# matteofox/MC-ALF

Hardware: AMD Instinct MI355X
Metric: component-pixel Voigt evals/s (sum_s ncomp_s * npix / t), logL batch on MI355X: `value` with the inputs resident in HBM when the timed region starts, `value_host_api` through the host-pointer entry with P in and logL out inside every step (higher is better)
Workload: dtype f64

## Files before the change

mc-alf_amd/csrc/kernels.hip:

```cpp
#include <hip/hip_runtime.h>

#include <cmath>

#include "kernel_args.h"
#include "voigt_device.h"

namespace mcalf {

__device__ __forceinline__ int xcd_raw() { return (int)(__builtin_amdgcn_s_getreg((3 << 11) | 20) & 15); }
__device__ __forceinline__ int xcd_id() { return (int)(__builtin_amdgcn_s_getreg((3 << 11) | 20) & (kXcds - 1)); }

__device__ __forceinline__ int tile_pos(int i) { return (i & 7) * kPlaneStride + (i >> 3); }

template <int kCtrl, int kRowMask = 0xF>
__device__ __forceinline__ double dpp_move(double v) {
    const unsigned long long u = __builtin_bit_cast(unsigned long long, v);
    const int lo = __builtin_amdgcn_update_dpp(0, (int)(unsigned)u, kCtrl, kRowMask, 0xF, false);
    const int hi = __builtin_amdgcn_update_dpp(0, (int)(unsigned)(u >> 32), kCtrl, kRowMask, 0xF, false);
    return __builtin_bit_cast(double, ((unsigned long long)(unsigned)hi << 32) | (unsigned)lo);
}

__device__ __forceinline__ double wave_sum_to_last(double v) {
    v += dpp_move<0x111>(v);
    v += dpp_move<0x112>(v);
// ... 507 lines not shown
        }
        __syncthreads();
        const int c = sClaim[0], cnt = sClaim[1];
        const bool ok = sClaim[2] != 0;
        __syncthreads();
        if (cnt == 0) {
            if (!rest && dedicated) { rest = true; continue; }
            break;
        }
        if (a.Pdev && ok) {
            const int perBlock = 8 * a.ndim, n = cnt * perBlock;
            for (int i0 = tid; i0 < n; i0 += 4 * kBlock) {
                double v[4];
                size_t at[4];
#pragma unroll
                for (int k = 0; k < 4; ++k) {
                    const int i = i0 + k * kBlock, blk = i / perBlock;
                    at[k] = (size_t)stream_row(x, 8 * (c + blk), nx) * a.ndim + (size_t)(i - blk * perBlock);
                    v[k] = (i < n && at[k] < (size_t)a.nrows * a.ndim) ? a.P[at[k]] : 0.0;
                }
#pragma unroll
                for (int k = 0; k < 4; ++k)
                    if (i0 + k * kBlock < n && at[k] < (size_t)a.nrows * a.ndim) a.Pdev[at[k]] = v[k];
            }
            stream_stores_done();
            __syncthreads();
        }
        for (int k = 0; k < cnt; ++k) {
            const int r = stream_row(x, 8 * (c + k) + wave, nx);
            if (r >= a.nrows) continue;
            SampleHdr* hdrp = reinterpret_cast<SampleHdr*>(reinterpret_cast<double*>(a.hdr) + (size_t)r * a.hdr_stride);
            if (ok) {
                setup_sample<kZeroPad>(as, (long)r, lane, a.recs + (size_t)r * a.rec_stride, a.taps + (size_t)r * a.tap_stride, true, hdrp, true,
                                       kSelfHalo, ends);
            } else if (lane == 0) {
                SampleHdr h;
                h.cont = 0.0; h.bot = 1.0; h.ncl = 0; h.n = 0; h.bad = 1; h.ngeneral = 0;
                *hdrp = h;
            }
        }
        stream_stores_done();
        if (lane < cnt) {
            const int r = stream_row(x, 8 * (c + lane) + wave, nx);
            if (r < a.nrows) __hip_atomic_store(a.ready + r, a.gen, __ATOMIC_RELAXED, __HIP_MEMORY_SCOPE_AGENT);
        }
    }
    __builtin_amdgcn_s_setprio(0);
    __syncthreads();
}

__device__ __forceinline__ void stream_exit(const KArgs& a, int tid) {
    if (tid != 0) return;
    stream_stores_done();
    if (atomicAdd(&a.sctl->exited, 1u) == gridDim.x - 1) {
        unsigned lo = ~0u, hi = 0u;
        for (int k = 0; k < kXcds; ++k) {
            const unsigned n = __hip_atomic_load(&a.sctl->arrive[k], __ATOMIC_RELAXED, __HIP_MEMORY_SCOPE_AGENT);
            lo = min(lo, n); hi = max(hi, n);
        }
        __hip_atomic_store(a.status + 2, lo, __ATOMIC_RELAXED, __HIP_MEMORY_SCOPE_SYSTEM);
        __hip_atomic_store(a.status + 3, hi, __ATOMIC_RELAXED, __HIP_MEMORY_SCOPE_SYSTEM);
        for (int k = 0; k < kXcds; ++k) {
            __hip_atomic_store(&a.sctl->arrive[k], 0u, __ATOMIC_RELAXED, __HIP_MEMORY_SCOPE_AGENT);
            __hip_atomic_store(&a.sctl->sq_eager[k], 0u, __ATOMIC_RELAXED, __HIP_MEMORY_SCOPE_AGENT);
            __hip_atomic_store(&a.sctl->sq_rest[k], 0u, __ATOMIC_RELAXED, __HIP_MEMORY_SCOPE_AGENT);
            __hip_atomic_store(&a.sctl->queue[k], 0u, __ATOMIC_RELAXED, __HIP_MEMORY_SCOPE_AGENT);
        }
        __hip_atomic_store(&a.sctl->exited, 0u, __ATOMIC_RELAXED, __HIP_MEMORY_SCOPE_AGENT);
        stream_stores_done();
        __hip_atomic_store(a.status + 1, a.gen, __ATOMIC_RELAXED, __HIP_MEMORY_SCOPE_SYSTEM);
    }
}

struct ItemLoads {
    double treg[(VT_NY * VT_NTOT + kBlock - 1) / kBlock];
    double rreg[2];
    double tapreg;
    double nu[kPpt];
    double nuNode;
    unsigned long long tileMask;
    SampleHdr hd;
};

template <bool kZeroPad, bool selfHalo, bool kInline, bool kCoh = false>
__device__ __forceinline__ void request_item(const KArgs& a, int w, int tid, ItemLoads& L) {
    asm volatile("" : "+v"(tid));
    constexpr int kTRegs = (VT_NY * VT_NTOT + kBlock - 1) / kBlock;
    constexpr int kRecRegs = 2;
    const int recTotal = a.ncl_cap * kRecStride, tapTotal = 2 * a.n_cap + 8;
    const int s = w / a.ntiles;
    const int tileIdx = w - s * a.ntiles;
#pragma unroll
    for (int i = 0; i < kTRegs; ++i) {
        const int idx = tid + i * kBlock;
        L.treg[i] = (idx < VT_NY * VT_NTOT) ? a.tabs[idx] : 0.0;
    }
    if (!kInline) {
        const double* gr = a.recs + (size_t)s * (kCoh ? a.rec_stride : recTotal);
        const double* gt = a.taps + (kCoh ? (size_t)s * a.tap_stride : (a.taps_shared ? 0 : (size_t)s * tapTotal));
        L.hd = kCoh ? *reinterpret_cast<const SampleHdr*>(reinterpret_cast<const double*>(a.hdr) + (size_t)s * a.hdr_stride) : a.hdr[s];
#pragma unroll
        for (int i = 0; i < kRecRegs; ++i) L.rreg[i] = (tid + i * kBlock < recTotal) ? gr[tid + i * kBlock] : 0.0;
        L.tapreg = (tid < tapTotal) ? gt[tid] : 0.0;
    }
    const int t0 = tileIdx * a.tile;
    const int ext0 = selfHalo ? 0 : t0 - a.n_cap;
    int npixW = a.npix;
    asm volatile("" : "+s"(npixW));
#pragma unroll
    for (int j = 0; j < kPpt; ++j) {
        int e = ext0 + tid + j * kBlock;
        if (!selfHalo && (e < 0 || e >= a.npix)) {
            if (kZeroPad) e = 0;
            else { e %= npixW; if (e < 0) e += npixW; }
        }
        L.nu[j] = a.nu[e];
    }
    L.nuNode = 0.0;
    L.tileMask = 0;
    if (kFarInterp && selfHalo && !kInline) {
        const int wv = tid >> 6, ln = tid & 63;
        L.nuNode = a.nu[kBlock * wv + 64 * (ln >> 3) + VT_INTERP_NODES[ln & 7]];
    } else if (kFarInterp) {
        const int wv = tid >> 6, ln = tid & 63;
        int e = ext0 + 64 * wv + kBlock * (ln >> 3) + VT_INTERP_NODES[ln & 7];
        if (!selfHalo && (e < 0 || e >= a.npix)) { e %= npixW; if (e < 0) e += npixW; }
        L.nuNode = a.nu[e];
        L.tileMask = a.segok[tileIdx];
    }
}

template <bool kZeroPad, bool kSelfHalo, int kLinesPerSync, bool kInline, bool kStream>
__device__ __forceinline__ void fused_items(const KArgs& a, double* smem) {
    double* sTab = smem;
    double* sRec = sTab + 2 * kLinesPerSync * kTabPad;
    double* sW = sRec + a.ncl_cap * kRecStride;
    double* sRed = sW + (2 * a.n_cap + 8);
    double* sWt = sRed + kRedDoubles;
    double* sF = sWt + 64 * VT_INODES;
    int* sNext = reinterpret_cast<int*>(sRed + 3 * kWaves);

    const int tid0 = threadIdx.x;
    double* sT = sF;
    constexpr int kTRegs = (VT_NY * VT_NTOT + kBlock - 1) / kBlock;
    constexpr int kRecRegs = 2;
    constexpr bool selfHalo = kSelfHalo;
    constexpr bool kPreMask = kSelfHalo && !kInline;
    static_assert(kLinesPerSync * kTabPad >= kBlock, "the node sums fit the idle half of the folded tables");
    if (kFarInterp) sWt[(tid0 & 7) * 64 + (tid0 >> 3)] = a.wtab[tid0];
    const int recTotal = a.ncl_cap * kRecStride, tapTotal = 2 * a.n_cap + 8;
    const int xcd = kStream ? xcd_id() : 0;
    const int nItems = kStream ? stream_rows_of(a.nrows, xcd, kXcds) * a.ntiles : a.nitems;

    constexpr bool kOrdered = kSelfHalo && !kInline && !kStream;
    auto item_of = [&](int t) -> int {
        if (kStream) { const int j = t / a.ntiles; return stream_row(xcd, j, kXcds) * a.ntiles + (t - j * a.ntiles); }
        return (kOrdered && a.order) ? a.order[t] : t;
    };
    constexpr bool kDeferTicket = kOrdered || kStream;
    int w;
    unsigned int* const queue = kStream ? &a.sctl->queue[xcd] : a.queue;
    const int firstTickets = kStream ? 0 : (int)gridDim.x;
    if (kStream) {
        if (tid0 == 0) sNext[0] = (int)atomicAdd(queue, 1u);
        __syncthreads();
        const int t = sNext[0];
        __syncthreads();
        if (t >= nItems) {
            stream_exit(a, tid0);
            return;
        }
        w = item_of(t);
        stream_wait_ready(a, w / a.ntiles, 0u);
    } else {
        w = item_of(blockIdx.x);
    }
    ItemLoads L;
    request_item<kZeroPad, kSelfHalo, kInline, kStream>(a, w, tid0, L);

    while (true) {
        int tid = tid0;
        asm volatile("" : "+v"(tid));
        const bool hasCoef = tid < VT_NTOT;
        const int coefPos = tid + (tid >= VT_Z0_OFF ? 1 : 0) + (tid >= VT_ZF_OFF ? 1 : 0);
        const bool coreCoef = tid < VT_NCORE;
        const int s = w / a.ntiles;
        const int tileIdx = w - s * a.ntiles;
        const int t0 = tileIdx * a.tile;
        const int tlen = min(a.tile, a.npix - t0);
        const int ext0 = selfHalo ? 0 : t0 - a.n_cap;
        const int extCount = tlen + 2 * a.n_cap;
        double nu[kPpt], tau[kPpt];
#pragma unroll
        for (int j = 0; j < kPpt; ++j) {
            const int idx = tid + j * kBlock;
            const int e = ext0 + idx;
            const bool zero = kZeroPad && !selfHalo && (e < 0 || e >= a.npix);
            nu[j] = L.nu[j];
            tau[j] = (zero && idx < extCount) ? INFINITY : 0.0;
        }
        const double nuNode = L.nuNode;
        double farNode = 0.0;
        unsigned long long segOk = 0;
        if (kFarInterp && !kPreMask) {
            const int wv = tid >> 6;
#pragma unroll
            for (int j = 0; j < kPpt; ++j) segOk |= ((L.tileMask >> (wv + 8 * j)) & 1ULL) << (8 * j);
            segOk = uniform64(segOk);
        }
        const int wvU = kPreMask ? __builtin_amdgcn_readfirstlane(tid >> 6) : 0;
        SampleHdr hd;
        SampleHdr* sHdr = reinterpret_cast<SampleHdr*>(sRed + 2 * kWaves);
        static_assert(sizeof(SampleHdr) <= kWaves * sizeof(double), "header fits the scratch slot");
        if (kInline) {
            if (tid < 64) setup_sample<kZeroPad>(a, s, tid, sRec, sW, true, sHdr, tileIdx == 0, false);
        } else {
            hd = L.hd;
#pragma unroll
            for (int i = 0; i < kRecRegs; ++i)
                if (tid + i * kBlock < recTotal) sRec[tid + i * kBlock] = L.rreg[i];
            if (recTotal > kRecRegs * kBlock) {
                const double* gr = a.recs + (size_t)s * (kStream ? a.rec_stride : recTotal);
                for (int i = tid + kRecRegs * kBlock; i < recTotal; i += kBlock) sRec[i] = gr[i];
            }
            if (tid < tapTotal) sW[tid] = L.tapreg;
            if (tapTotal > kBlock) {
                const double* gt = a.taps + (kStream ? (size_t)s * a.tap_stride : (a.taps_shared ? 0 : (size_t)s * tapTotal));
                for (int i = tid + kBlock; i < tapTotal; i += kBlock) sW[i] = gt[i];
            }
        }
#pragma unroll
        for (int i = 0; i < kTRegs; ++i) {
            const int idx = tid + i * kBlock;
            if (idx < VT_NY * VT_NTOT) sT[idx] = L.treg[i];
        }
        int tHeld = nItems, wHeld = 0;
        unsigned stHeld = 0u;
        if (tid == 0) {
            tHeld = a.persist ? firstTickets + (int)atomicAdd(queue, 1u) : nItems;
            if (kOrdered) wHeld = (tHeld < nItems) ? item_of(tHeld) : 0;
            else if (kStream) {
                wHeld = (tHeld < nItems) ? item_of(tHeld) : 0;
                if (tHeld < nItems) stHeld = __hip_atomic_load(a.ready + wHeld / a.ntiles, __ATOMIC_RELAXED, __HIP_MEMORY_SCOPE_AGENT);
            } else { sNext[0] = tHeld; sNext[1] = tHeld; }
        }

        __syncthreads();
        if (kInline) hd = *sHdr;
        const double cont = kStream ? __builtin_bit_cast(double, uniform64(__builtin_bit_cast(unsigned long long, hd.cont))) : hd.cont;
        const double bot = kStream ? __builtin_bit_cast(double, uniform64(__builtin_bit_cast(unsigned long long, hd.bot))) : hd.bot;
        const int ncl = kStream ? min(max(hd.ncl, 0), a.ncl_cap) : hd.ncl, n = kStream ? min(max(hd.n, 0), a.n_cap) : hd.n;
        const bool bad = hd.bad != 0;
        const int shift = a.n_cap - n;
        int tNext = 0, wNext = 0;
        if (!kDeferTicket) {
            tNext = __builtin_amdgcn_readfirstlane(sNext[0]);
            wNext = __builtin_amdgcn_readfirstlane(sNext[1]);
        }
        int buf = 0;
        const int ncl_run = ncl;
        for (int cl0 = 0; cl0 < ncl_run; cl0 += kLinesPerSync) {
            if (4 * cl0 < ncl_run) __builtin_amdgcn_s_setprio(3);
            else if (4 * cl0 < 2 * ncl_run) __builtin_amdgcn_s_setprio(2);
            else if (4 * cl0 < 3 * ncl_run) __builtin_amdgcn_s_setprio(1);
            else __builtin_amdgcn_s_setprio(0);
            double* tabs = sTab + buf * (kLinesPerSync * kTabPad);
            if (hasCoef) {
                double Tn[VT_NY];
#pragma unroll
                for (int nn = 0; nn < VT_NY; ++nn) Tn[nn] = sT[nn * VT_NTOT + tid];
                double fy[kLinesPerSync], fs[kLinesPerSync], fc[kLinesPerSync];
#pragma unroll
                for (int l = 0; l < kLinesPerSync; ++l) {
                    const double* rec = sRec + min(cl0 + l, ncl_run - 1) * kRecStride;
                    fy[l] = rec[3];
                    fs[l] = coreCoef ? rec[4] : rec[5];
                    fc[l] = Tn[VT_NY - 1];
                }
#pragma unroll
                for (int nn = VT_NY - 2; nn >= 0; --nn) {
#pragma unroll
                    for (int l = 0; l < kLinesPerSync; ++l) fc[l] = fma(fc[l], fy[l], Tn[nn]);
                    __builtin_amdgcn_sched_barrier(0);
                }
#pragma unroll
                for (int l = 0; l < kLinesPerSync; ++l) tabs[l * kTabPad + coefPos] = fc[l] * fs[l];
            } else if (tid >= kBlock - 64 && tid < kBlock - 64 + 3) {
                const int which = tid - (kBlock - 64);
                const int src = (which == 0) ? 7 : which - 1;
#pragma unroll
                for (int l = 0; l < kLinesPerSync; ++l)
                    tabs[l * kTabPad + kLineLds + which] = sRec[min(cl0 + l, ncl_run - 1) * kRecStride + src];
            }
            __syncthreads();
            buf ^= 1;
            const int lmax = __builtin_amdgcn_readfirstlane(min(kLinesPerSync, ncl_run - cl0));
#pragma unroll 1
            for (int l = 0; l < lmax; ++l) eval_line<kPreMask>(tabs + l * kTabPad, nu, tau, nuNode, farNode, segOk, wvU);
        }
        if (hd.ngeneral > 0 && ncl_run > 0) eval_general_lines(sRec, ncl, nu, tau);
        __builtin_amdgcn_s_setprio(0);
        double wrow[VT_INODES];
        double* sFar = kPreMask ? sTab + buf * (kLinesPerSync * kTabPad) + 8 * (tid >> 6) : sTab + (tid >> 6) * 64;
        constexpr int kFarSlot = kPreMask ? 64 : 8;
        if (kFarInterp) {
            if (kPreMask) sTab[buf * (kLinesPerSync * kTabPad) + tid] = farNode;
            __syncthreads();
            if (!kPreMask) sFar[tid & 63] = farNode;
#pragma unroll
            for (int k = 0; k < VT_INODES; ++k) wrow[k] = sWt[k * 64 + (tid & 63)];
        }
        const int extTight = tlen + 2 * n;
        const int posBody = tile_pos(selfHalo ? tid + n : tid - shift);
        const int posLow = tile_pos(tid + n + a.npix), posHigh = tile_pos(tid + n - a.npix);
        static_assert(kBlock % 8 == 0, "tile_pos(i + kBlock) == tile_pos(i) + kBlock / 8");
        static_assert(kPpt % 2 == 0, "pixels are processed in pairs");
#pragma unroll
        for (int j0 = 0; j0 < kPpt; j0 += 2) {
            double fl[2];
#pragma unroll
            for (int jj = 0; jj < 2; ++jj) {
                const int j = j0 + jj;
                double tj = tau[j];
                if (kFarInterp) {
                    double add = 0.0;
#pragma unroll
                    for (int k = 0; k < VT_INODES; ++k) add = fma(wrow[k], sFar[kFarSlot * j + k], add);
                    tj += add;
                }
                fl[jj] = exp_neg(tj);
            }
#pragma unroll
            for (int jj = 0; jj < 2; ++jj) {
                const int j = j0 + jj;
                if (selfHalo) {
                    const int p = tid + j * kBlock;
                    if (p < a.npix) {
                        sF[posBody + (kBlock / 8) * j] = fl[jj];
                        if (j * kBlock < n && p < n) sF[posLow + (kBlock / 8) * j] = kZeroPad ? 0.0 : fl[jj];
                        if ((j + 1) * kBlock > a.npix - n && p >= a.npix - n) sF[posHigh + (kBlock / 8) * j] = kZeroPad ? 0.0 : fl[jj];
                    }
                } else {
                    const int pos = tid + j * kBlock - shift;
                    if (pos >= 0 && pos < extTight) sF[posBody + (kBlock / 8) * j] = fl[jj];
                }
            }
            __builtin_amdgcn_sched_barrier(0);
            asm volatile("" ::: "memory");
        }
        if (tid < kTileSlack) {
            double zero = 0.0;
            asm volatile("" : "+v"(zero));
            sF[tile_pos(extTight + tid)] = zero;
        }
        if (kDeferTicket && tid == 0) { sNext[0] = tHeld; sNext[1] = wHeld; if (kStream) sNext[2] = (int)stHeld; }
        __syncthreads();
        if (kDeferTicket) {
            tNext = __builtin_amdgcn_readfirstlane(sNext[0]);
            wNext = __builtin_amdgcn_readfirstlane(sNext[1]);
        }
        unsigned stampNext = 0u;
        if (kStream) stampNext = (unsigned)__builtin_amdgcn_readfirstlane(sNext[2]);

        double acc = 0.0, nnz = 0.0, c4 = 0.0, c5 = 0.0;
        const int base = 8 * tid;
        const bool reduces = (a.mode == kModeLogL || a.mode == kModeChi2);
        if (base < tlen) {
            const size_t o0 = (size_t)(t0 + base);
            double ob[8], is2[8], lg[8];
#pragma unroll
            for (int m = 0; m < 8; ++m) { ob[m] = a.obj[o0 + m]; is2[m] = a.ispec2[o0 + m]; lg[m] = a.lgis[o0 + m]; }
            double win[8], top[8];
            const double* fp = sF + tid;
#pragma unroll
            for (int m = 0; m < 8; ++m) { win[m] = fp[m * kPlaneStride]; top[m] = 0.0; }
            const double* wp = sW;
            const int ntaps = 2 * n + 1;
            for (int q0 = 0; q0 + 8 <= ntaps; q0 += 8) {
                ++fp;
#pragma unroll
                for (int r = 0; r < 8; ++r) {
                    const double wgt = wp[r];
#pragma unroll
                    for (int m = 0; m < 8; ++m) top[m] = fma(win[(m + r) & 7], wgt, top[m]);
                    win[r] = fp[r * kPlaneStride];
                }
                wp += 8;
            }
            {
                const int rem = ntaps & 7;
                ++fp;
#pragma unroll
                for (int r = 0; r < 7; ++r) {
                    if (r >= rem) break;
                    const double wgt = wp[r];
#pragma unroll
                    for (int m = 0; m < 8; ++m) top[m] = fma(win[(m + r) & 7], wgt, top[m]);
                    win[r] = fp[r * kPlaneStride];
                }
            }
            const double ibot = 1.0 / bot;
            const bool plainLogL = !kZeroPad && a.mode == kModeLogL && !a.asymm && a.model == nullptr;
            if (plainLogL) {
                if (!bad) {
#pragma unroll
                    for (int m = 0; m < 8; ++m) {
                        double mval = top[m] * ibot;
                        mval *= cont;
                        const double d = ob[m] - mval;
                        double term = is2[m] * (d * d);
                        term = (term - lg[m]) + a.log2pi;
                        acc += (base + m < tlen && !isnan(term)) ? term : 0.0;
                    }
                }
            } else if (!kZeroPad && a.mode != kModeLogL && a.mode != kModeChi2 && a.model != nullptr) {
                double* mrow = a.model + (size_t)s * a.npix + t0 + base;
#pragma unroll
                for (int m = 0; m < 8; ++m) {
                    double mval = top[m] * ibot;
                    mval *= cont;
                    if (bad) mval = NAN;
                    if (base + m < tlen) mrow[m] = mval;
                }
            } else
#pragma unroll
            for (int m = 0; m < 8; ++m) {
                const int i = base + m;
                const bool live = i < tlen;
                const int pix = t0 + i;
                double mval = kZeroPad ? top[m] : top[m] * ibot;
                if (kZeroPad && (pix < n || pix >= a.npix - n)) mval = sF[tile_pos(min(i, tlen - 1) + n)];
                mval *= cont;
                if (bad) mval = NAN;
                if (a.model && live) a.model[(size_t)s * a.npix + pix] = mval;
                if (reduces) {
                    const double d = ob[m] - mval;
                    double term = is2[m] * (d * d);
                    if (a.mode == kModeLogL) term = (term - lg[m]) + a.log2pi;
// ... 393 lines not shown
```

mc-alf_amd/csrc/voigt_tables.h:

```cpp
#pragma once
#define VT_XCORE 8.0
#define VT_XMID 6.0
#define VT_NINT 32
#define VT_CDEG 11
#define VT_CSTRIDE 12
#define VT_WDEG 10
#define VT_NY 7
#define VT_NCORE 384
#define VT_Z1_OFF 384
#define VT_Z0_OFF 395
#define VT_ZF_OFF 406
#define VT_FDEG 6
#define VT_XFAR 16.0
#define VT_NTOT 413
#define VT_Z1_A 164.57142857142858
#define VT_Z1_B -3.5714285714285716
static const double VT_T_HOST[7 * 413] = {
  0.9844964370054085, -0.03076551365641901, -0.014902045677327391, 0.0004757037430598439, 0.00011270579635484074, -3.677559621145527e-06,
  -5.678553713961873e-07, 1.8952744614798227e-08, 2.1440963963345023e-09, -7.325115457232298e-11, -6.422962611576024e-12, 2.2474713691397446e-13,
  0.8688150562628432, -0.08145141152464154, -0.009757200338889547, 0.0011533647139719456, 4.9196142166143476e-05, -8.130957127553065e-06,
  -1.2918371174934012e-07, 3.8029053146936205e-08, 5.898971028117496e-11, -1.3265677473511572e-10, 1.0426041036144699e-12, 3.653232648815428e-13,
  0.676633846161729, -0.10572403846277015, -0.00231271334137368, 0.0012217458871837071, -2.9656375731835644e-05, -6.709150053097754e-06,
  3.291777105791387e-07, 2.260384547161342e-08, -1.7272758883395457e-09, -4.8497436982902636e-11, 6.105826908641806e-12, 5.057301034298833e-14,
  0.4650431881340563, -0.10172819740432482, 0.003860221776503226, 0.0007781942184250338, -7.271547894705505e-05, -1.6824116614028525e-06,
// ... 395 lines not shown
  1.435414873550603e-13, -5.103605919981534e-15, 1.7513373694376256e-16, -5.865613630420488e-18, 1.9409157244517318e-19, -6.353636259510203e-21,
  4.31831629856487e-06, -4.72216761988616e-07, 3.048267446779884e-08, -1.5179075691664099e-09, 6.460480208346226e-11, -2.4774455768866935e-12,
  8.833169218731325e-14, -2.98922443357065e-15, 9.741564419850537e-17, -3.0904469420178764e-18, 9.652594096568941e-20, -2.9721382407051117e-21,
  3.484629904536954e-06, -3.6661608331952456e-07, 2.2746900863582402e-08, -1.0875485527103187e-09, 4.4391089159693915e-11, -1.63045121965053e-12,
  5.560076090322122e-14, -1.796811793402878e-15, 5.581989435011656e-17, -1.684728724278554e-18, 4.993084472643356e-20, -1.4553146815359711e-21,
  2.834346377850398e-06, -2.873790598500714e-07, 1.7168789116439216e-08, -7.896563006293831e-10, 3.097585387353248e-11, -1.0922007351057677e-12,
  3.5713221726129627e-14, -1.1052006801958649e-15, 3.283187304844695e-17, -9.46044014870273e-19, 2.671392727690264e-20, -7.405057288054136e-22,
  0.0, 0.0, 0.0, 0.0, 0.0, 0.0,
  0.0, 0.0, 0.0, 0.0, 0.0, 0.0,
  0.0, 0.0, 0.0, 0.0, 0.0, 0.0,
  0.0, 0.0, 0.0, 0.0, 0.0, 0.0,
  0.0, 0.0, 0.0, 0.0, 0.0,
  0.14885988589579738, -0.03477843985261595, -0.0157381368971371, 0.0016130405865366448, 0.00035626070372722873, -2.7430388551944085e-05,
  -3.939286363686594e-06, 2.625002348230792e-07, 2.755023480353477e-08, -1.6906187315983065e-09, -1.366203413068305e-10, 7.987041827130155e-12,
  0.033864732371850156, -0.06978361945159416, -0.00043284794139333767, 0.0029211773086501233, -5.832021936193879e-05, -4.454989131932472e-05,
  1.364343784163328e-06, 3.794943643247482e-07, -1.4343276467083794e-08, -2.156432961859019e-09, 9.358232312466788e-11, 8.906280733075687e-12,
  -0.08629196937074665, -0.04147823702053563, 0.012678671417137794, 0.001067912406213029, -0.0003388716895089491, -6.09639105371196e-06,
  4.04166411499425e-06, -3.5783630174467544e-08, -2.8619580792459878e-08, 7.142492004805167e-10, 1.3645304436121685e-10, -5.132478571524964e-12,
  -0.11536023630779482, 0.011452735364309245, 0.011364882915703605, -0.0013058866861147792, -0.00019494876530501754, 2.8933487938577027e-05,
  1.1789216790356292e-06, -2.9517596237456357e-07, -4.821742124182374e-10, 1.8052262322619204e-09, -3.613663655085657e-11, -7.404266853332872e-12,
  -0.059597218330350234, 0.03741546052327415, 0.0012568966188086798, -0.001676811579815797, 8.844229956190641e-05, 2.122530158246559e-05,
  -2.008336761151288e-06, -1.0881952122853087e-07, 1.839393718241207e-08, 8.643331467088222e-11, -9.720483350336873e-11, 2.0740786975324863e-12,
  0.008803278910407443, 0.026433697961397065, -0.005506150467945236, -0.0004704910072737846, 0.00016948322258020237, -4.300549554782163e-06,
  -1.6956098210100986e-06, 1.2166428360595196e-07, 7.073390990511971e-09, -1.0093827136413826e-09, -2.5094211931859098e-12, 4.6148328438141815e-12,
  0.03836461348341036, 0.003576526516677748, -0.004922611548454827, 0.0005175817089910177, 6.280681592509694e-05, -1.3190267993321402e-05,
  1.734292985643098e-07, 1.0770514914752105e-07, -6.726900429596657e-09, -3.508071945937582e-10, 4.87201114999256e-11, -2.0574355549416114e-13,
  0.030573727665031906, -0.008874243785771044, -0.0012641005760717632, 0.0005672758727520629, -3.6850284098258104e-05, -5.408971381344243e-06,
  8.448187781254041e-07, -8.278283823181273e-09, -5.643748958757977e-09, 3.4422008856721023e-10, 1.3345378764402225e-11, -2.1099390278587156e-12,
  0.011596102780949292, -0.008581706926194232, 0.0010111921606068058, 0.00017850584348439631, -4.7407623634555986e-05, 2.247906204077142e-06,
  3.4417913124666015e-07, -4.619132165916281e-08, 5.702893417406741e-10, 2.4700437425323496e-10, -1.5854248606037316e-11, -3.514862964307029e-13,
  -0.0007647140463144033, -0.0036856220790373873, 0.0011778096535299753, -7.954057396798336e-05, -1.579810980756273e-05, 3.1188470087819575e-06,
  -1.2761588802207266e-07, -1.7022290324847334e-08, 2.1891470374106154e-09, -4.098099307328359e-11, -8.958787274627695e-12, 6.627586797229027e-13,
  -0.004223825484327467, -0.0002149215012355374, 0.0005325020299403835, -0.00010752975649815364, 5.161084358593728e-06, 1.0027601244028458e-06,
  -1.688143555402584e-07, 6.873126957878992e-09, 6.609274921229773e-10, -8.995140435821706e-11, 2.388759009373724e-12, 2.6285413825957874e-13,
  -0.00327903101854847, 0.0008412563010667681, 5.63175344576683e-05, -4.8545088508287285e-05, 7.403003379825596e-06, -3.056647278729244e-07,
  -4.8210003207758624e-08, 7.679283875242856e-09, -3.4017860803147953e-10, -1.9496217536531654e-11, 3.155888312915918e-12, -1.1650150402880712e-13,
  -0.0016531387782024655, 0.0006902338366796043, -8.881053858691549e-05, -5.631998771263517e-06, 3.1814967562738572e-06, -4.091088876860956e-07,
  1.6814744059024985e-08, 1.7761133891819736e-09, -2.9544590835822156e-10, 1.4852432980036618e-11, 3.920987679467979e-13, -9.419053722391747e-14,
  -0.0006339211123832547, 0.00034024369905524615, -7.420518887193266e-05, 6.693388576280134e-06, 3.272974604336404e-07, -1.5981564305246208e-07,
  1.8723795428457852e-08, -8.299604395755084e-10, -4.830397872396267e-11, 9.571420699088113e-12, -5.49103638853042e-13, -1.2922913902890553e-15,
  -0.00019550064097057147, 0.00012462480822260393, -3.508773361972092e-05, 5.4067191883443816e-06, -4.0259105928333616e-07, -1.151035778428637e-08,
  6.35156569328965e-09, -7.195300030148162e-10, 3.543298552435304e-11, 8.044804152020773e-13, -2.5828231235973135e-13, 1.7423174116355718e-14,
  -4.9834340217112394e-05, 3.6284919016206255e-05, -1.2124876687244389e-05, 2.403453137909344e-06, -2.979095092916644e-07, 2.0166012176231872e-08,
  1.5757494055164956e-10, -2.018610132613121e-10, 2.330253613306998e-11, -1.2815532615868693e-12, 1.4045613319287405e-15, 5.622039291910619e-15,
  -1.0668055523932667e-05, 8.66782158197365e-06, -3.3025269302782607e-06, 7.740843997001548e-07, -1.2216565933155704e-07, 1.3101598495519118e-08,
  -8.520225560392942e-10, 8.542615836035427e-12, 5.080081523102568e-12, -6.339989505473961e-13, 3.864593358132985e-14, -7.372504993772694e-16,
  -1.9376664443186664e-06, 1.7297221353120294e-06, -7.340095254002962e-07, 1.95535883831295e-07, -3.626349499655905e-08, 4.877391342421659e-09,
  -4.73588527811759e-10, 3.045008071273107e-11, -7.27572877906246e-13, -9.66222203305686e-14, 1.4452554895662955e-14, -9.857318636193877e-16,
  -3.0074754699070465e-07, 2.9168239471429725e-07, -1.3573462149136092e-07, 4.016095225361806e-08, -8.427745078171065e-09, 1.3214011687483672e-09,
  -1.580770679974741e-10, 1.4312724025027593e-11, -9.219419337716663e-13, 3.146820302071138e-14, 1.2259281589912468e-15, -2.6798654642919357e-16,
  -4.009677779598275e-08, 4.189281740302217e-08, -2.114285053339468e-08, 6.843748970774943e-09, -1.5896692067484913e-09, 2.8054829123814086e-10,
  -3.877140520065936e-11, 4.2454836708416285e-12, -3.655202422765074e-13, 2.3699780272002766e-14, -9.729984635002326e-16, 2.7315814579897956e-19,
  -4.610092307514334e-09, 5.154090667561649e-09, -2.7976104877896577e-09, 9.800590346696507e-10, -2.4835616353279716e-10, 4.8327844556350796e-11,
  -7.474261628008081e-12, 9.365579778491905e-13, -9.577218797197436e-14, 7.943712403995941e-15, -5.204508494993516e-16, 2.4224328685277084e-17,
  -4.5849637617332825e-10, 5.455400790626808e-10, -3.1638669949359725e-10, 1.1898403918001854e-10, -3.255588719060251e-11, 6.890269118169591e-12,
  -1.1700978427223898e-12, 1.6309659856737949e-13, -1.890503583960406e-14, 1.8317837577331534e-15, -1.4916048455723096e-16, 9.761627407228198e-18,
  -3.954157026202408e-11, 4.984563549766568e-11, -3.0722853217399735e-11, 1.232443596429488e-11, -3.6127425820740895e-12, 8.23514553933956e-13,
  -1.5161548943704811e-13, 2.3105619833616022e-14, -2.9611158365803135e-15, 3.2233009167850805e-16, -3.037617490806172e-17, 2.383138971412457e-18,
  -2.9630013077703494e-12, 3.942049096046695e-12, -2.570864038024017e-12, 1.0944001391257198e-12, -3.415954117439896e-13, 8.324365308764029e-14,
  -1.6463295900869558e-14, 2.711097117541265e-15, -3.7819732307161197e-16, 4.5256759102087554e-17, -4.775802110994971e-18, 4.253421136945533e-19,
  -1.9323623970909245e-13, 2.70435052681158e-13, -1.859166236710121e-13, 8.3626816058698e-14, -2.7655967551298147e-14, 7.162971545992829e-15,
  -1.5111677172901885e-15, 2.6661155425712197e-16, -4.0051074367464014e-17, 5.19583801727527e-18, -6.02424858896022e-19, 5.927185736077348e-20,
  -1.0983164786323914e-14, 1.6122704237248577e-14, -1.1646496312778252e-14, 5.5154218130080454e-15, -1.9245858617377777e-15, 5.272833383841798e-16,
  -1.1800819868148526e-16, 2.215989266374078e-17, -3.556441251832404e-18, 4.953318880115225e-19, -6.232225824841678e-20, 6.6637035285320976e-21,
  -5.447045369546799e-16, 8.365813444871777e-16, -6.332168693974528e-16, 3.1473092293615505e-16, -1.1547722643135578e-16, 3.3334166791174696e-17,
  -7.878553309525776e-18, 1.5664795039961508e-18, -2.669414929708172e-19, 3.96257198180321e-20, -5.363045315139608e-21, 6.163164424683842e-22,
  -2.3595467229899835e-17, 3.7829947809322154e-17, -2.9929357353916795e-17, 1.5570779738291112e-17, -5.989097961517763e-18, 1.8154595147777993e-18,
  -4.514375842199792e-19, 9.463325275413155e-20, -1.7038749040945045e-20, 2.680514875082888e-21, -3.876918460856498e-22, 4.7501518914093874e-23,
  -8.935330899809956e-19, 1.492460466188387e-18, -1.2314924336333308e-18, 6.690127735371166e-19, -2.690564989849601e-19, 8.539809013828966e-20,
  -2.2270250360827628e-20, 4.904406874608974e-21, -9.292193320721401e-22, 1.5421849771618395e-22, -2.3714604065498257e-23, 3.0788921095651268e-24,
  -2.9603218606998054e-20, 5.141940763369629e-20, -4.4164415111337273e-20, 2.5000237766877018e-20, -1.0488435036840861e-20, 3.476983901493843e-21,
  -9.483048459724605e-22, 2.1872670575424266e-22, -4.345947015580951e-23, 7.58059619782052e-24, -1.2342651569113333e-24, 1.689748833928469e-25,
  -8.586275914270748e-22, 1.5483635558064507e-21, -1.381871657417956e-21, 8.135491154918345e-22, -3.553189614048274e-22, 1.227537597708343e-22,
  -3.49303322672239e-23, 8.415986098000906e-24, -1.7484899757885403e-24, 3.195235886211903e-25, -5.489924655446723e-26, 7.8936572800312e-27,
  -2.1815535551971927e-23, 4.078127743456147e-23, -3.775799728551532e-23, 2.3079465021452525e-23, -1.0474453454469908e-23, 3.7637041546714724e-24,
  -1.1150211725925169e-24, 2.7998342275890994e-25, -6.066745882420897e-26, 1.158334970980848e-26, -2.0942457510973782e-27, 3.15198136675935e-28,
  0.0, 0.0, 0.0, 0.0, 0.0, 0.0,
  0.0, 0.0, 0.0, 0.0, 0.0, 0.0,
  0.0, 0.0, 0.0, 0.0, 0.0, 0.0,
  0.0, 0.0, 0.0, 0.0, 0.0, 0.0,
  0.0, 0.0, 0.0, 0.0, 0.0,
};
#define VT_INODES 8
static const int VT_INTERP_NODES[8] = {0, 3, 12, 24, 39, 51, 60, 63};
static const double VT_INTERP_W_HOST[64 * 8] = {
  1.0, 0.0, 0.0, 0.0, 0.0, 0.0, 0.0, 0.0,
  0.5413865891050592, 0.5247650710185003, -0.09569964958927814, 0.04446170055452177, -0.02691102928300002, 0.02105392290964119, -0.017788646475203403, 0.008732041759759019,
  0.21723909658126556, 0.8422779007799945, -0.08448187089271438, 0.03730368325132843, -0.022180568419708793, 0.017241198141370283, -0.014522032772068871, 0.007122593330533297,
  0.0, 1.0, 0.0, 0.0, 0.0, 0.0, 0.0, 0.0,
  -0.13387071968529243, 1.0380852298403378, 0.13015208858292318, -0.05057338299222158, 0.02889907599555519, -0.022153546992837992, 0.01853723624714889, -0.009075980995613046,
  -0.20430017703680256, 0.9901390159020474, 0.28375024588444797, -0.10155271957969718, 0.0567500491768896, -0.043179385243285566, 0.036005055123710814, -0.017612084227310566,
  -0.22798157724628312, 0.8839285714285714, 0.4432975113122172, -0.14354395604395603, 0.0782967032967033, -0.05910633484162896, 0.049107142857142856, -0.023998060762766647,
  -0.21872838333743683, 0.7420456338224009, 0.5954272657519114, -0.17012207592911754, 0.09037735283734369, -0.06766218928998993, 0.05600344406206799, -0.027341047917179603,
  -0.18780443132900165, 0.5825232185783771, 0.7303505662794508, -0.1773708518107238, 0.09154624609585743, -0.06793958756087914, 0.056011847940228565, -0.02731700819330933,
  -0.14423076923076922, 0.4194078947368421, 0.8413461538461539, -0.16346153846153846, 0.08173076923076923, -0.06009615384615385, 0.049342105263157895, -0.02403846153846154,
  -0.09506999574477183, 0.26328908595983175, 0.9242916252963927, -0.12826904187786675, 0.06192298573414257, -0.0450873963559216, 0.036860472034376444, -0.017937735046183362,
  -0.04568887454387333, 0.12178690133350446, 0.9772342610772907, -0.07302409862995139, 0.03390404579247743, -0.02443085652693227, 0.019883575727919097, -0.009664954230434744,
  0.0, 0.0, 1.0, 0.0, 0.0, 0.0, 0.0, 0.0,
  0.039316709765753584, -0.09908500627807898, 0.9938390524121044, 0.08776760462860143, -0.037132448112100605, 0.026153659274002747, -0.021081916229378505, 0.01022234453909593,
  0.07061191663890769, -0.17422110851736872, 0.9611066431406879, 0.18672929066733365, -0.07469171626693345, 0.051951710440037185, -0.04166156942806643, 0.020174833325402194,
  0.09308338720103426, -0.22556390977443608, 0.9049773755656109, 0.29304029304029305, -0.10989010989010989, 0.07541478129713423, -0.06015037593984962, 0.029088558500323207,
  0.10661036248061181, -0.2543685841642668, 0.8291917081825363, 0.4027502582600891, -0.14008704635133534, 0.09476476664943273, -0.07515435441216974, 0.036292889355101894,
  0.11160499689306273, -0.26271928153335633, 0.7378330350152481, 0.5119657793983354, -0.162898202535834, 0.10850485809047766, -0.08553651026667415, 0.04124532493874058,
  0.10888009049773756, -0.2532894736842105, 0.6351338612368024, 0.6169871794871795, -0.1762820512820513, 0.11547888386123681, -0.09046052631578948, 0.04355203619909502,
  0.09953233869961055, -0.22913173804806178, 0.5253095653590557, 0.7144210088883157, -0.17860525222207893, 0.11491146742229343, -0.08941726362851192, 0.04297987352937728,
  0.0848403235234511, -0.19349547470260775, 0.4124182393501095, 0.8012697221659271, -0.16868836256124778, 0.10643051338067341, -0.0822355767486083, 0.039460615592302836,
  0.0661764705882353, -0.14967105263157895, 0.3002450980392157, 0.875, -0.14583333333333334, 0.0900735294117647, -0.06907894736842106, 0.03308823529411765,
  0.04493219590956216, -0.10085888112294147, 0.1922099491686826, 0.9335911816764583, -0.10983425666781862, 0.0662792928167871, -0.05042944056147074, 0.024109958780740674,
  0.022455466657838964, -0.05006190220254187, 0.09129621545232508, 0.9755652736905595, -0.060972829605659966, 0.03586637035627057, -0.027060487677049657, 0.012911893328257405,
  0.0, 0.0, 0.0, 1.0, 0.0, 0.0, 0.0, 0.0,
  -0.021314675847476622, 0.046955177056343035, -0.07970231353223096, 1.0065263594641738, 0.0718947399617267, -0.03985115676611548, 0.02951468272112991, -0.01402281305755041,
  -0.040533074226489864, 0.08882648531861585, -0.14636943470676894, 0.9953121560060288, 0.1531249470778506, -0.08196688343579062, 0.06008850477435778, -0.028482700807803688,
  -0.056884292178409825, 0.12406015037593984, -0.19909502262443438, 0.967032967032967, 0.24175824175824176, -0.1244343891402715, 0.09022556390977443, -0.04266321913380737,
  -0.06979401799058056, 0.15153873099147808, -0.23749353344017, 0.9228320156532319, 0.3355752784193571, -0.16521289282794432, 0.11838963358709226, -0.05583521439246445,
  -0.07888878002046726, 0.17057968662320333, -0.2616735677149486, 0.8642704122242303, 0.43213520611211514, -0.20220230232518754, 0.1430668339420415, -0.06728748884098679,
  -0.08399321266968326, 0.18092105263157895, -0.27220022624434387, 0.7932692307692307, 0.5288461538461539, -0.23331447963800905, 0.16282894736842105, -0.07635746606334842,
  -0.08512111538013256, 0.18269572727734593, -0.2700479830042217, 0.7120448857988867, 0.6230392750740259, -0.25654558385401066, 0.17639587461260986, -0.08246108052450342,
  -0.08246108052450342, 0.17639587461260986, -0.25654558385401066, 0.6230392750740259, 0.7120448857988867, -0.2700479830042217, 0.18269572727734593, -0.08512111538013256,
  -0.07635746606334842, 0.16282894736842105, -0.23331447963800905, 0.5288461538461539, 0.7932692307692307, -0.27220022624434387, 0.18092105263157895, -0.08399321266968326,
  -0.06728748884098679, 0.1430668339420415, -0.20220230232518754, 0.43213520611211514, 0.8642704122242303, -0.2616735677149486, 0.17057968662320333, -0.07888878002046726,
  -0.05583521439246445, 0.11838963358709226, -0.16521289282794432, 0.3355752784193571, 0.9228320156532319, -0.23749353344017, 0.15153873099147808, -0.06979401799058056,
  -0.04266321913380737, 0.09022556390977443, -0.1244343891402715, 0.24175824175824176, 0.967032967032967, -0.19909502262443438, 0.12406015037593984, -0.056884292178409825,
  -0.028482700807803688, 0.06008850477435778, -0.08196688343579062, 0.1531249470778506, 0.9953121560060288, -0.14636943470676894, 0.08882648531861585, -0.040533074226489864,
  -0.01402281305755041, 0.02951468272112991, -0.03985115676611548, 0.0718947399617267, 1.0065263594641738, -0.07970231353223096, 0.046955177056343035, -0.021314675847476622,
  0.0, 0.0, 0.0, 0.0, 1.0, 0.0, 0.0, 0.0,
  0.012911893328257405, -0.027060487677049657, 0.03586637035627057, -0.060972829605659966, 0.9755652736905595, 0.09129621545232508, -0.05006190220254187, 0.022455466657838964,
  0.024109958780740674, -0.05042944056147074, 0.0662792928167871, -0.10983425666781862, 0.9335911816764583, 0.1922099491686826, -0.10085888112294147, 0.04493219590956216,
  0.03308823529411765, -0.06907894736842106, 0.0900735294117647, -0.14583333333333334, 0.875, 0.3002450980392157, -0.14967105263157895, 0.0661764705882353,
  0.039460615592302836, -0.0822355767486083, 0.10643051338067341, -0.16868836256124778, 0.8012697221659271, 0.4124182393501095, -0.19349547470260775, 0.0848403235234511,
  0.04297987352937728, -0.08941726362851192, 0.11491146742229343, -0.17860525222207893, 0.7144210088883157, 0.5253095653590557, -0.22913173804806178, 0.09953233869961055,
  0.04355203619909502, -0.09046052631578948, 0.11547888386123681, -0.1762820512820513, 0.6169871794871795, 0.6351338612368024, -0.2532894736842105, 0.10888009049773756,
  0.04124532493874058, -0.08553651026667415, 0.10850485809047766, -0.162898202535834, 0.5119657793983354, 0.7378330350152481, -0.26271928153335633, 0.11160499689306273,
  0.036292889355101894, -0.07515435441216974, 0.09476476664943273, -0.14008704635133534, 0.4027502582600891, 0.8291917081825363, -0.2543685841642668, 0.10661036248061181,
  0.029088558500323207, -0.06015037593984962, 0.07541478129713423, -0.10989010989010989, 0.29304029304029305, 0.9049773755656109, -0.22556390977443608, 0.09308338720103426,
  0.020174833325402194, -0.04166156942806643, 0.051951710440037185, -0.07469171626693345, 0.18672929066733365, 0.9611066431406879, -0.17422110851736872, 0.07061191663890769,
  0.01022234453909593, -0.021081916229378505, 0.026153659274002747, -0.037132448112100605, 0.08776760462860143, 0.9938390524121044, -0.09908500627807898, 0.039316709765753584,
  0.0, 0.0, 0.0, 0.0, 0.0, 1.0, 0.0, 0.0,
  -0.009664954230434744, 0.019883575727919097, -0.02443085652693227, 0.03390404579247743, -0.07302409862995139, 0.9772342610772907, 0.12178690133350446, -0.04568887454387333,
  -0.017937735046183362, 0.036860472034376444, -0.0450873963559216, 0.06192298573414257, -0.12826904187786675, 0.9242916252963927, 0.26328908595983175, -0.09506999574477183,
  -0.02403846153846154, 0.049342105263157895, -0.06009615384615385, 0.08173076923076923, -0.16346153846153846, 0.8413461538461539, 0.4194078947368421, -0.14423076923076922,
  -0.02731700819330933, 0.056011847940228565, -0.06793958756087914, 0.09154624609585743, -0.1773708518107238, 0.7303505662794508, 0.5825232185783771, -0.18780443132900165,
  -0.027341047917179603, 0.05600344406206799, -0.06766218928998993, 0.09037735283734369, -0.17012207592911754, 0.5954272657519114, 0.7420456338224009, -0.21872838333743683,
  -0.023998060762766647, 0.049107142857142856, -0.05910633484162896, 0.0782967032967033, -0.14354395604395603, 0.4432975113122172, 0.8839285714285714, -0.22798157724628312,
  -0.017612084227310566, 0.036005055123710814, -0.043179385243285566, 0.0567500491768896, -0.10155271957969718, 0.28375024588444797, 0.9901390159020474, -0.20430017703680256,
  -0.009075980995613046, 0.01853723624714889, -0.022153546992837992, 0.02889907599555519, -0.05057338299222158, 0.13015208858292318, 1.0380852298403378, -0.13387071968529243,
  0.0, 0.0, 0.0, 0.0, 0.0, 0.0, 1.0, 0.0,
  0.007122593330533297, -0.014522032772068871, 0.017241198141370283, -0.022180568419708793, 0.03730368325132843, -0.08448187089271438, 0.8422779007799945, 0.21723909658126556,
  0.008732041759759019, -0.017788646475203403, 0.02105392290964119, -0.02691102928300002, 0.04446170055452177, -0.09569964958927814, 0.5247650710185003, 0.5413865891050592,
  0.0, 0.0, 0.0, 0.0, 0.0, 0.0, 0.0, 1.0,
};
```

Baseline: 625.5 billion.

## Defer persistent ticket resolution, clamp prefetch loads, pack interp node offsets

The atomic ticket fetch is issued early but its result is resolved only after the line evaluation, so the atomic latency is hidden behind compute. Prefetch loads use clamped indices instead of predicated loads, and self-halo mode skips the item-to-sample division. Interpolation node offsets become a packed constexpr word rather than a table lookup, and header fields are made wave-uniform with readfirstlane. The changes add some register pressure and compiler barriers, and the clamped loads read duplicate addresses.

```diff
diff --git a/mc-alf_amd/csrc/kernels.hip b/mc-alf_amd/csrc/kernels.hip
--- a/mc-alf_amd/csrc/kernels.hip
+++ b/mc-alf_amd/csrc/kernels.hip
@@ -613,26 +613,32 @@
     SampleHdr hd;
 };
 
+constexpr unsigned long long interp_node_word() {
+    unsigned long long v = 0;
+    for (int k = 0; k < VT_INODES; ++k) v |= (unsigned long long)VT_INTERP_NODES[k] << (8 * k);
+    return v;
+}
+constexpr unsigned long long kNodeWord = interp_node_word();
+static_assert(VT_INODES == 8 && kNodeWord == 0x3F3C3327180C0300ULL, "node offsets 0, 3, 12, 24, 39, 51, 60, 63: one byte each");
+__device__ __forceinline__ int interp_node(int k) { return (int)((kNodeWord >> (8 * (k & 7))) & 0xFFu); }
+
 template <bool kZeroPad, bool selfHalo, bool kInline, bool kCoh = false>
 __device__ __forceinline__ void request_item(const KArgs& a, int w, int tid, ItemLoads& L) {
     asm volatile("" : "+v"(tid));
     constexpr int kTRegs = (VT_NY * VT_NTOT + kBlock - 1) / kBlock;
     constexpr int kRecRegs = 2;
     const int recTotal = a.ncl_cap * kRecStride, tapTotal = 2 * a.n_cap + 8;
-    const int s = w / a.ntiles;
-    const int tileIdx = w - s * a.ntiles;
-#pragma unroll
-    for (int i = 0; i < kTRegs; ++i) {
-        const int idx = tid + i * kBlock;
-        L.treg[i] = (idx < VT_NY * VT_NTOT) ? a.tabs[idx] : 0.0;
-    }
+    const int s = selfHalo ? w : w / a.ntiles;
+    const int tileIdx = selfHalo ? 0 : w - s * a.ntiles;
+#pragma unroll
+    for (int i = 0; i < kTRegs; ++i) L.treg[i] = a.tabs[min(tid + i * kBlock, VT_NY * VT_NTOT - 1)];
     if (!kInline) {
         const double* gr = a.recs + (size_t)s * (kCoh ? a.rec_stride : recTotal);
         const double* gt = a.taps + (kCoh ? (size_t)s * a.tap_stride : (a.taps_shared ? 0 : (size_t)s * tapTotal));
         L.hd = kCoh ? *reinterpret_cast<const SampleHdr*>(reinterpret_cast<const double*>(a.hdr) + (size_t)s * a.hdr_stride) : a.hdr[s];
 #pragma unroll
-        for (int i = 0; i < kRecRegs; ++i) L.rreg[i] = (tid + i * kBlock < recTotal) ? gr[tid + i * kBlock] : 0.0;
-        L.tapreg = (tid < tapTotal) ? gt[tid] : 0.0;
+        for (int i = 0; i < kRecRegs; ++i) L.rreg[i] = gr[min(tid + i * kBlock, recTotal - 1)];
+        L.tapreg = gt[min(tid, tapTotal - 1)];
     }
     const int t0 = tileIdx * a.tile;
     const int ext0 = selfHalo ? 0 : t0 - a.n_cap;
@@ -651,10 +657,10 @@
     L.tileMask = 0;
     if (kFarInterp && selfHalo && !kInline) {
         const int wv = tid >> 6, ln = tid & 63;
-        L.nuNode = a.nu[kBlock * wv + 64 * (ln >> 3) + VT_INTERP_NODES[ln & 7]];
+        L.nuNode = a.nu[kBlock * wv + 64 * (ln >> 3) + interp_node(ln)];
     } else if (kFarInterp) {
         const int wv = tid >> 6, ln = tid & 63;
-        int e = ext0 + 64 * wv + kBlock * (ln >> 3) + VT_INTERP_NODES[ln & 7];
+        int e = ext0 + 64 * wv + kBlock * (ln >> 3) + interp_node(ln);
         if (!selfHalo && (e < 0 || e >= a.npix)) { e %= npixW; if (e < 0) e += npixW; }
         L.nuNode = a.nu[e];
         L.tileMask = a.segok[tileIdx];
@@ -715,8 +721,8 @@
         const bool hasCoef = tid < VT_NTOT;
         const int coefPos = tid + (tid >= VT_Z0_OFF ? 1 : 0) + (tid >= VT_ZF_OFF ? 1 : 0);
         const bool coreCoef = tid < VT_NCORE;
-        const int s = w / a.ntiles;
-        const int tileIdx = w - s * a.ntiles;
+        const int s = selfHalo ? w : w / a.ntiles;
+        const int tileIdx = selfHalo ? 0 : w - s * a.ntiles;
         const int t0 = tileIdx * a.tile;
         const int tlen = min(a.tile, a.npix - t0);
         const int ext0 = selfHalo ? 0 : t0 - a.n_cap;
@@ -730,7 +736,7 @@
             nu[j] = L.nu[j];
             tau[j] = (zero && idx < extCount) ? INFINITY : 0.0;
         }
-        const double nuNode = L.nuNode;
+        double nuNode = L.nuNode;
         double farNode = 0.0;
         unsigned long long segOk = 0;
         if (kFarInterp && !kPreMask) {
@@ -747,6 +753,11 @@
             if (tid < 64) setup_sample<kZeroPad>(a, s, tid, sRec, sW, true, sHdr, tileIdx == 0, false);
         } else {
             hd = L.hd;
+            asm volatile("" : "+v"(hd.ncl), "+v"(hd.n), "+v"(hd.bad), "+v"(hd.ngeneral));
+            hd.ncl = __builtin_amdgcn_readfirstlane(hd.ncl);
+            hd.n = __builtin_amdgcn_readfirstlane(hd.n);
+            hd.bad = __builtin_amdgcn_readfirstlane(hd.bad);
+            hd.ngeneral = __builtin_amdgcn_readfirstlane(hd.ngeneral);
 #pragma unroll
             for (int i = 0; i < kRecRegs; ++i)
                 if (tid + i * kBlock < recTotal) sRec[tid + i * kBlock] = L.rreg[i];
@@ -765,16 +776,32 @@
             const int idx = tid + i * kBlock;
             if (idx < VT_NY * VT_NTOT) sT[idx] = L.treg[i];
         }
-        int tHeld = nItems, wHeld = 0;
-        unsigned stHeld = 0u;
+        int wHeld = 0;
+        unsigned stHeld = 0u, tRaw = 0u;
+        if (kDeferTicket) {
+            asm volatile("" : "+v"(nuNode));
+#pragma unroll
+            for (int j = 0; j < kPpt; ++j) asm volatile("" : "+v"(nu[j]));
+        }
         if (tid == 0) {
-            tHeld = a.persist ? firstTickets + (int)atomicAdd(queue, 1u) : nItems;
-            if (kOrdered) wHeld = (tHeld < nItems) ? item_of(tHeld) : 0;
-            else if (kStream) {
+            if (kDeferTicket) {
+                int qoff = 0;
+                asm volatile("" : "+v"(qoff));
+                if (a.persist) tRaw = atomicAdd(queue + qoff, 1u);
+            } else {
+                const int tHeld = a.persist ? firstTickets + (int)atomicAdd(queue, 1u) : nItems;
+                sNext[0] = tHeld; sNext[1] = tHeld;
+            }
+        }
+        auto resolve_ticket = [&]() {
+            asm volatile("" : "+v"(tRaw));
+            if (tid == 0) {
+                const int tHeld = a.persist ? firstTickets + (int)tRaw : nItems;
+                sNext[0] = tHeld;
                 wHeld = (tHeld < nItems) ? item_of(tHeld) : 0;
-                if (tHeld < nItems) stHeld = __hip_atomic_load(a.ready + wHeld / a.ntiles, __ATOMIC_RELAXED, __HIP_MEMORY_SCOPE_AGENT);
-            } else { sNext[0] = tHeld; sNext[1] = tHeld; }
-        }
+                if (kStream && tHeld < nItems) stHeld = __hip_atomic_load(a.ready + wHeld / a.ntiles, __ATOMIC_RELAXED, __HIP_MEMORY_SCOPE_AGENT);
+            }
+        };
 
         __syncthreads();
         if (kInline) hd = *sHdr;
@@ -831,6 +858,7 @@
         }
         if (hd.ngeneral > 0 && ncl_run > 0) eval_general_lines(sRec, ncl, nu, tau);
         __builtin_amdgcn_s_setprio(0);
+        if (kDeferTicket) resolve_ticket();
         double wrow[VT_INODES];
         double* sFar = kPreMask ? sTab + buf * (kLinesPerSync * kTabPad) + 8 * (tid >> 6) : sTab + (tid >> 6) * 64;
         constexpr int kFarSlot = kPreMask ? 64 : 8;
@@ -884,7 +912,7 @@
             asm volatile("" : "+v"(zero));
             sF[tile_pos(extTight + tid)] = zero;
         }
-        if (kDeferTicket && tid == 0) { sNext[0] = tHeld; sNext[1] = wHeld; if (kStream) sNext[2] = (int)stHeld; }
+        if (kDeferTicket && tid == 0) { sNext[1] = wHeld; if (kStream) sNext[2] = (int)stHeld; }
         __syncthreads();
         if (kDeferTicket) {
             tNext = __builtin_amdgcn_readfirstlane(sNext[0]);
diff --git a/mc-alf_amd/csrc/voigt_tables.h b/mc-alf_amd/csrc/voigt_tables.h
--- a/mc-alf_amd/csrc/voigt_tables.h
+++ b/mc-alf_amd/csrc/voigt_tables.h
@@ -501,7 +501,7 @@
   0.0, 0.0, 0.0, 0.0, 0.0,
 };
 #define VT_INODES 8
-static const int VT_INTERP_NODES[8] = {0, 3, 12, 24, 39, 51, 60, 63};
+static constexpr int VT_INTERP_NODES[8] = {0, 3, 12, 24, 39, 51, 60, 63};
 static const double VT_INTERP_W_HOST[64 * 8] = {
   1.0, 0.0, 0.0, 0.0, 0.0, 0.0, 0.0, 0.0,
   0.5413865891050592, 0.5247650710185003, -0.09569964958927814, 0.04446170055452177, -0.02691102928300002, 0.02105392290964119, -0.017788646475203403, 0.008732041759759019,
```

New measurement: 642.2 billion, median of 6. +2.7%, better.
